# wkgcass/vproxy

Measured on AMD Instinct MI355X. Metric: device-resident GB/s, batched IPv4+TCP checksum, 1500B pkts, 1/2/4/8 GPU, higher is better.
Workload: dtype u8

## Files before the change

vproxy_amd/csrc/tcp_build.hip:

```cpp
#include <hip/hip_runtime.h>
#include <stdint.h>

#include "device_common.h"
#include "internal.h"
#include "tcp_build.h"
#include "team_move.h"

namespace vpcsum {

__global__ __launch_bounds__(256) void k_tcp_build(uint8_t* __restrict__ dst, uint64_t dst_len,
                                                  const uint8_t* __restrict__ src, uint64_t src_len,
                                                  const vpcsum_tcphdr_t* __restrict__ hdrs, uint32_t n_hdr,
                                                  const vpcsum_tcpseg_t* __restrict__ segs, uint32_t n,
                                                  uint32_t* __restrict__ frame_len_out, uint32_t* __restrict__ out,
                                                  uint8_t* __restrict__ status) {
    const uint32_t tid = blockIdx.x * 256u + threadIdx.x;
    const uint32_t i = tid >> 3;
    const uint32_t tl = threadIdx.x & 7u;
    if (i >= n) return;

    const u32x4a4_t ra = *(gu32x4a4_t*)(segs + i);
    const u32x4a4_t rb = *(gu32x4a4_t*)((const uint8_t*)(segs + i) + 16);
    const uint64_t frame_off = ((uint64_t)ra.y << 32) | ra.x, data_off = ((uint64_t)ra.w << 32) | ra.z;
    const uint32_t seq = rb.x, hdr = rb.y, frame_cap = rb.z;
    const uint32_t data_len = rb.w & 0xffffu, flags = (rb.w >> 16) & 0xffu, rsv = rb.w >> 24;

    bool ok = tcp_build_seg_ok(hdr, n_hdr, flags, rsv);
    uint32_t t[16] = {0, 0, 0, 0, 0, 0, 0, 0, 0, 0, 0, 0, 0, 0, 0, 0};
    if (ok) {
        const uint8_t* hp = (const uint8_t*)(hdrs + hdr);
        const u32x4a4_t h0 = *(gu32x4a4_t*)hp, h1 = *(gu32x4a4_t*)(hp + 16), h2 = *(gu32x4a4_t*)(hp + 32),
                        h3 = *(gu32x4a4_t*)(hp + 48);
        t[0] = h0.x; t[1] = h0.y; t[2] = h0.z; t[3] = h0.w;
        t[4] = h1.x; t[5] = h1.y; t[6] = h1.z; t[7] = h1.w;
        t[8] = h2.x; t[9] = h2.y; t[10] = h2.z; t[11] = h2.w;
        t[12] = h3.x; t[13] = h3.y; t[14] = h3.z; t[15] = h3.w;
        ok = tcp_build_hdr_ok(t) && tcp_build_fits(t, frame_off, data_off, frame_cap, data_len, dst_len, src_len);
    }
    if (!ok) {
        if (tl == 0) {
            frame_len_out[i] = 0u;
            if (out) out[i] = 0u;
            if (status) status[i] = (uint8_t)VPCSUM_S_BAD_DESC;
        }
        return;
    }

    const bool v4 = tb_l3_ver(t) == 4;
    const uint32_t l2 = tb_l2_len(t), H = tcp_build_header_len(t);
    uint8_t* const frame = dst + frame_off;
    uint8_t* const pay = frame + H;

    const Span sp = make_span((uintptr_t)pay, (uintptr_t)(src + data_off), data_len, 0u);
    const uint32_t ng = data_len ? (sp.hi + 15u) >> 4 : 0u;
    const uint64_t acc = move_groups<false>(sp, tl, ng);
    uint32_t ps = fold32(team_sum<8>(fold64(acc)));
    if ((uintptr_t)pay & 1u) ps = bswap16(ps);

    TcpBuildWords w;
    tcp_build_words(t, seq, data_len, flags, w);
    const uint32_t ip_field = v4 ? 0xffffu - fold64(tcp_build_ip_header_sum(w)) : 0u;
    const uint32_t l4_field = 0xffffu - fold64(tcp_build_l4_header_sum(t, w, data_len) + ps);
    tcp_build_set_sums(w, v4, ip_field, l4_field);

    if (tl == 0) {
        if (l2) {
            store_piece_any<14>(frame, Piece{w.eth[0], w.eth[1], w.eth[2], w.eth[3], 0u});
        }
        frame_len_out[i] = H + data_len;
        if (out) out[i] = bswap16(ip_field) | (bswap16(l4_field) << 16);
        if (status) status[i] = (uint8_t)VPCSUM_S_DONE;
    } else if (tl == 1) {
        store_piece_any<20>(frame + l2, Piece{w.ip[0], w.ip[1], w.ip[2], w.ip[3], w.ip[4]});
    } else if (tl == 2 && !v4) {
        store_piece_any<20>(frame + l2 + 20u, Piece{w.ip[5], w.ip[6], w.ip[7], w.ip[8], w.ip[9]});
    } else if (tl == (v4 ? 2u : 3u)) {
        store_piece_any<20>(frame + l2 + (v4 ? 20u : 40u), Piece{w.tcp[0], w.tcp[1], w.tcp[2], w.tcp[3], w.tcp[4]});
    }
}

hipError_t launch_tcp_build(uint8_t* dst, uint64_t dst_len, const uint8_t* src, uint64_t src_len,
                            const vpcsum_tcphdr_t* hdrs, uint32_t n_hdr, const vpcsum_tcpseg_t* segs, uint32_t n,
                            uint32_t* frame_len_out, uint32_t* out, uint8_t* status, hipStream_t stream) {
    if (n == 0) return hipSuccess;
    const uint32_t g = (n + 31u) / 32u;
    hipLaunchKernelGGL(k_tcp_build, dim3(g), dim3(256), 0, stream, dst, dst_len, src, src_len, hdrs, n_hdr, segs, n,
                       frame_len_out, out, status);
    return hipGetLastError();
}

}
```

vproxy_amd/csrc/tcp_recv.hip:

```cpp
#include <hip/hip_runtime.h>
#include <stdint.h>

#include "device_common.h"
#include "internal.h"
#include "tcp_recv.h"
#include "team_move.h"

namespace vpcsum {

namespace {

__device__ __forceinline__ uint32_t load_shifted(uintptr_t p) {
    const uint32_t sh = (uint32_t)p & 3u;
    const uintptr_t a = p - sh;
    const uint32_t lo = *(gu32_t*)a;
    const uint32_t hi = sh ? *(gu32_t*)(a + 4) : 0u;
    return alignbyte(hi, lo, sh);
}

struct Desc {
    uint64_t l3_off;
    uint32_t l3_len, l4_off, l3_ver, l4_proto, flags;
};
__device__ __forceinline__ Desc load_desc(const vpcsum_desc_t* d) {
    const u32x4a4_t v = *(gu32x4a4_t*)d;
    Desc r;
    r.l3_off = ((uint64_t)v.y << 32) | v.x;
    r.l3_len = v.z & 0xffffu;
    r.l4_off = v.z >> 16;
    r.l3_ver = v.w & 0xffu;
    r.l4_proto = (v.w >> 8) & 0xffu;
    r.flags = (v.w >> 16) & 0xffu;
    return r;
}

}

__global__ __launch_bounds__(256) void k_tcp_recv(const uint8_t* __restrict__ arena, uint64_t arena_len,
                                                 const vpcsum_desc_t* __restrict__ desc,
                                                 const vpcsum_tcprx_t* __restrict__ rx, uint32_t n,
                                                 uint8_t* __restrict__ dst, uint64_t dst_len,
                                                 uint32_t* __restrict__ stored_out, uint32_t* __restrict__ out,
                                                 uint8_t* __restrict__ status) {
    const uint32_t tid = blockIdx.x * 256u + threadIdx.x;
    const uint32_t i = tid >> 3;
    const uint32_t tl = threadIdx.x & 7u;
    if (i >= n) return;

    const Desc d = load_desc(desc + i);
    const u32x4a4_t ra = *(gu32x4a4_t*)(rx + i);
    const uint64_t dst_off = ((uint64_t)ra.y << 32) | ra.x;
    const uint32_t dst_cap = ra.z, skip = ra.w & 0xffffu, ops = (ra.w >> 16) & 0xffu, rsv = ra.w >> 24;

    bool ok = tcp_recv_desc_ok(d.l3_off, d.l3_len, d.l4_off, d.l3_ver, d.l4_proto, d.flags, arena_len) &&
              tcp_recv_ops_ok(ops, rsv);
    const uint32_t seg_len = d.l3_len - d.l4_off;
    const uintptr_t l3 = (uintptr_t)arena + d.l3_off, seg = l3 + d.l4_off;
    uint32_t hlen = 0, data_len = 0, stored = 0;
    if (ok) {
        const uint32_t b12 = *(gu8_t*)(seg + 12);
        ok = tcp_recv_hdr_ok(seg_len, b12, &hlen, &data_len) &&
             tcp_recv_store_ok(data_len, skip, ops, dst_off, dst_cap, dst_len, &stored);
    }
    if (!ok) {
        if (tl == 0) {
            stored_out[i] = 0u;
            if (out) out[i] = 0u;
            if (status) status[i] = (uint8_t)VPCSUM_S_BAD_DESC;
        }
        return;
    }
    const uint32_t field = (uint32_t) * (gu8_t*)(seg + 16) | ((uint32_t) * (gu8_t*)(seg + 17) << 8);

    const uintptr_t v0 = stored ? (uintptr_t)dst + dst_off - (hlen + skip) : seg;
    const Span sp = make_span(v0, seg, seg_len, stored ? hlen + skip : seg_len);
    const uint32_t ng = (sp.hi + 15u) >> 4;
    const uint64_t acc = move_groups<true>(sp, tl, ng);

    const bool v4 = d.l3_ver == 4u;
    uint32_t ph = 0;
    if (tl < (v4 ? 2u : 8u)) {
        const uint32_t w = load_shifted(l3 + (v4 ? 12u : 8u) + 4u * tl);
        ph = (w & 0xffffu) + (w >> 16);
    }
    uint32_t ipw = 0;
    if (tl == 7u && (d.flags & VPCSUM_F_IP)) {
        const uint32_t sh = (uint32_t)l3 & 3u, nw = d.l4_off >> 2;
        const uintptr_t a = l3 - sh;
        uint64_t ipacc = 0;
        uint32_t cur = *(gu32_t*)a, ip_field = 0;
        for (uint32_t j = 0; j < nw; ++j) {
            const uint32_t nxt = (sh || j + 1u < nw) ? *(gu32_t*)(a + 4u * j + 4u) : 0u;
            uint32_t w = alignbyte(nxt, cur, sh);
            cur = nxt;
            if (j == 2u) {
                ip_field = w >> 16;
                w &= 0xffffu;
            }
            ipacc += w;
        }
        const uint32_t ipc = 0xffffu - bswap16(fold64(ipacc));
        ipw = ipc | (bswap16(ip_field) == ipc ? 0x10000u : 0u);
    }

    uint32_t ps = fold32(team_sum<8>(fold64(acc)));
    if (v0 & 1u) ps = bswap16(ps);
    ph = team_sum<8>(ph);
    ipw = team_sum<8>(ipw);
    if (tl == 0) {
        const uint64_t total = (uint64_t)ps + ph + (6u << 8) + bswap16(seg_len) + (0xffffu - field);
        const uint32_t l4c = 0xffffu - bswap16(fold64(total));
        uint32_t st = VPCSUM_S_DONE;
        if (bswap16(field) == l4c) st |= VPCSUM_S_L4_OK;
        if (ipw & 0x10000u) st |= VPCSUM_S_IP_OK;
        stored_out[i] = stored;
        if (out) out[i] = (ipw & 0xffffu) | (l4c << 16);
        if (status) status[i] = (uint8_t)st;
    }
}

__global__ __launch_bounds__(256) void k_tcp_digest(const uint8_t* __restrict__ arena, uint64_t arena_len,
                                                   const vpcsum_desc_t* __restrict__ desc, uint32_t n,
                                                   vpcsum_tcpinfo_t* __restrict__ info) {
    const uint32_t i = blockIdx.x * 256u + threadIdx.x;
    if (i >= n) return;
    const Desc d = load_desc(desc + i);
    u32x4_t o;
    o.x = o.y = o.z = o.w = 0u;
    if (tcp_recv_desc_ok(d.l3_off, d.l3_len, d.l4_off, d.l3_ver, d.l4_proto, d.flags, arena_len)) {
        const uintptr_t seg = (uintptr_t)arena + d.l3_off + d.l4_off;
        const uint32_t sh = (uint32_t)seg & 3u;
        const uintptr_t a = seg - sh;
        const u32x4a4_t v = *(gu32x4a4_t*)a;
        const uint32_t w4 = sh ? *(gu32_t*)(a + 16) : 0u;
        const uint32_t d1 = alignbyte(v.z, v.y, sh), d2 = alignbyte(v.w, v.z, sh),
                       d3 = alignbyte(w4, v.w, sh);
        uint32_t hlen = 0, data_len = 0;
        if (tcp_recv_hdr_ok(d.l3_len - d.l4_off, d3 & 0xffu, &hlen, &data_len)) {
            o.x = __builtin_bswap32(d1);
            o.y = __builtin_bswap32(d2);
            o.z = bswap16(d3 >> 16) | (data_len << 16);
            o.w = hlen | (((d3 >> 8) & 0x3fu) << 8);
        }
    }
    *(gwu32x4_t*)(info + i) = o;
}

hipError_t launch_tcp_recv(const uint8_t* arena, uint64_t arena_len, const vpcsum_desc_t* desc, const vpcsum_tcprx_t* rx,
                           uint32_t n, uint8_t* dst, uint64_t dst_len, uint32_t* stored, uint32_t* out, uint8_t* status,
                           hipStream_t stream) {
    if (n == 0) return hipSuccess;
    const uint32_t g = (n + 31u) / 32u;
    hipLaunchKernelGGL(k_tcp_recv, dim3(g), dim3(256), 0, stream, arena, arena_len, desc, rx, n, dst, dst_len, stored, out,
                       status);
    return hipGetLastError();
}

hipError_t launch_tcp_digest(const uint8_t* arena, uint64_t arena_len, const vpcsum_desc_t* desc, uint32_t n,
                             vpcsum_tcpinfo_t* info, hipStream_t stream) {
    if (n == 0) return hipSuccess;
    hipLaunchKernelGGL(k_tcp_digest, dim3((n + 255u) / 256u), dim3(256), 0, stream, arena, arena_len, desc, n, info);
    return hipGetLastError();
}

}
```

vproxy_amd/csrc/team_move.h:

```cpp
#pragma once
#include <stdint.h>

#include "device_common.h"

#define VPC_TM_FN __host__ __device__ __forceinline__

namespace vpcsum {

#ifdef __HIP_DEVICE_COMPILE__
#define VPC_TM_LOAD(T, a) __builtin_nontemporal_load((T*)(a))
VPC_TM_FN uint32_t alignbyte(uint32_t hi, uint32_t lo, uint32_t sh) { return __builtin_amdgcn_alignbyte(hi, lo, sh); }
#else
#define VPC_TM_LOAD(T, a) (*(T*)(a))
VPC_TM_FN uint32_t alignbyte(uint32_t hi, uint32_t lo, uint32_t sh) {
    return (uint32_t)((((uint64_t)hi << 32) | lo) >> ((sh & 3u) * 8u));
}
#endif

struct Span {
    uintptr_t sa;
    uintptr_t pd;
    uint32_t sh;
    uint32_t lo, hi;
    uint32_t s_lo, s_hi;
    uint32_t k_lo, k_hi;
};

VPC_TM_FN Span make_span(uintptr_t v0, uintptr_t seg, uint32_t seg_len, uint32_t store_from) {
    Span sp;
    sp.lo = (uint32_t)v0 & 15u;
    sp.hi = sp.lo + seg_len;
    sp.pd = v0 - sp.lo;
    sp.s_lo = sp.lo + store_from;
    sp.s_hi = sp.hi;
    const uintptr_t s0 = seg - sp.lo;
    sp.sh = (uint32_t)s0 & 3u;
    sp.sa = s0 - sp.sh;
    sp.k_lo = (sp.lo + sp.sh) >> 2;
    sp.k_hi = (sp.lo + sp.sh + seg_len - 1u) >> 2;
    return sp;
}

struct Group {
    uint32_t w0, w1, w2, w3, w4;
};

VPC_TM_FN bool group_inner(const Span& sp, uint32_t g) { return g * 16u >= sp.lo && g * 16u + 16u <= sp.hi; }

VPC_TM_FN Group load_group(const Span& sp, uint32_t g) {
    Group r;
    const uintptr_t q = sp.sa + (size_t)g * 16u;
    if (group_inner(sp, g)) {
        const u32x4a4_t v = VPC_TM_LOAD(gu32x4a4_t, q);
        r.w0 = v.x; r.w1 = v.y; r.w2 = v.z; r.w3 = v.w;
        r.w4 = sp.sh ? VPC_TM_LOAD(gu32_t, q + 16) : 0u;
    } else {
        const uint32_t k = g * 4u;
        r.w0 = (k >= sp.k_lo && k <= sp.k_hi) ? VPC_TM_LOAD(gu32_t, q) : 0u;
        r.w1 = (k + 1 >= sp.k_lo && k + 1 <= sp.k_hi) ? VPC_TM_LOAD(gu32_t, q + 4) : 0u;
        r.w2 = (k + 2 >= sp.k_lo && k + 2 <= sp.k_hi) ? VPC_TM_LOAD(gu32_t, q + 8) : 0u;
        r.w3 = (k + 3 >= sp.k_lo && k + 3 <= sp.k_hi) ? VPC_TM_LOAD(gu32_t, q + 12) : 0u;
        r.w4 = (k + 4 >= sp.k_lo && k + 4 <= sp.k_hi) ? VPC_TM_LOAD(gu32_t, q + 16) : 0u;
    }
    return r;
}

VPC_TM_FN void store_partial(uintptr_t a, uint32_t v, uint32_t m) {
    if ((m & 0xffffu) == 0xffffu) {
        *(gwu16_t*)a = (uint16_t)v;
    } else {
        if (m & 0xffu) *(gwu8_t*)a = (uint8_t)v;
        if (m & 0xff00u) *(gwu8_t*)(a + 1) = (uint8_t)(v >> 8);
    }
    if ((m >> 16) == 0xffffu) {
        *(gwu16_t*)(a + 2) = (uint16_t)(v >> 16);
    } else {
        if (m & 0xff0000u) *(gwu8_t*)(a + 2) = (uint8_t)(v >> 16);
        if (m & 0xff000000u) *(gwu8_t*)(a + 3) = (uint8_t)(v >> 24);
    }
}

template <bool SUB>
VPC_TM_FN void emit_group(const Span& sp, uint32_t g, const Group& r, uint64_t& acc) {
    uint32_t d0 = alignbyte(r.w1, r.w0, sp.sh);
    uint32_t d1 = alignbyte(r.w2, r.w1, sp.sh);
    uint32_t d2 = alignbyte(r.w3, r.w2, sp.sh);
    uint32_t d3 = alignbyte(r.w4, r.w3, sp.sh);
    const uint32_t rel = g * 16u;
    const uintptr_t p = sp.pd + (size_t)rel;
    const uint32_t s_lo = SUB ? sp.s_lo : sp.lo, s_hi = SUB ? sp.s_hi : sp.hi;
    if (rel >= s_lo && rel + 16u <= s_hi) {
        acc += (uint64_t)d0 + d1 + d2 + d3;
        u32x4_t o;
        o.x = d0; o.y = d1; o.z = d2; o.w = d3;
        *(gwu32x4_t*)p = o;
        return;
    }
    if (!SUB || !group_inner(sp, g)) {
        const int lo = (int)sp.lo, hi = (int)sp.hi;
        d0 &= bmask((int)rel, lo, hi);
        d1 &= bmask((int)rel + 4, lo, hi);
        d2 &= bmask((int)rel + 8, lo, hi);
        d3 &= bmask((int)rel + 12, lo, hi);
    }
    acc += (uint64_t)d0 + d1 + d2 + d3;
    if (!SUB || (rel + 16u > s_lo && rel < s_hi)) {
        const int lo = (int)s_lo, hi = (int)s_hi;
        const uint32_t m0 = bmask((int)rel, lo, hi), m1 = bmask((int)rel + 4, lo, hi), m2 = bmask((int)rel + 8, lo, hi),
                       m3 = bmask((int)rel + 12, lo, hi);
        if (m0 == 0xffffffffu) *(gwu32_t*)p = d0; else if (m0) store_partial(p, d0, m0);
        if (m1 == 0xffffffffu) *(gwu32_t*)(p + 4) = d1; else if (m1) store_partial(p + 4, d1, m1);
        if (m2 == 0xffffffffu) *(gwu32_t*)(p + 8) = d2; else if (m2) store_partial(p + 8, d2, m2);
        if (m3 == 0xffffffffu) *(gwu32_t*)(p + 12) = d3; else if (m3) store_partial(p + 12, d3, m3);
    }
}

template <bool SUB>
VPC_TM_FN uint64_t move_groups(const Span& sp, uint32_t tl, uint32_t ng) {
    uint64_t acc = 0;
    for (uint32_t g = tl; g < ng; g += 16u) {
        const bool two = g + 8u < ng;
        const Group a = load_group(sp, g);
        Group b = {0u, 0u, 0u, 0u, 0u};
        if (two) b = load_group(sp, g + 8u);
        emit_group<SUB>(sp, g, a, acc);
        if (two) emit_group<SUB>(sp, g + 8u, b, acc);
    }
    return acc;
}


struct Piece {
    uint32_t w0, w1, w2, w3, w4;
};

template <int K>
__device__ __forceinline__ uint32_t piece_word(const Piece w) {
    return K == 0 ? w.w0 : K == 1 ? w.w1 : K == 2 ? w.w2 : K == 3 ? w.w3 : K == 4 ? w.w4 : 0u;
}

template <int POS>
__device__ __forceinline__ uint32_t piece_bytes(const Piece w) {
    constexpr int k = POS >> 2, sh = (POS & 3) * 8;
    const uint32_t lo = piece_word<k>(w);
    if constexpr (sh == 0) return lo;
    else return (lo >> sh) | (piece_word<k + 1>(w) << (32 - sh));
}

template <int R, int NB, int POS = 0>
__device__ __forceinline__ void store_piece(uint8_t* p, const Piece w) {
    if constexpr (POS < NB) {
        constexpr int a = (R + POS) & 3;
        if constexpr (a == 0 && NB - POS >= 4) {
            *(gwu32_t*)(p + POS) = piece_bytes<POS>(w);
            store_piece<R, NB, POS + 4>(p, w);
        } else if constexpr ((a & 1) == 0 && NB - POS >= 2) {
            *(gwu16_t*)(p + POS) = (uint16_t)piece_bytes<POS>(w);
            store_piece<R, NB, POS + 2>(p, w);
        } else {
            *(gwu8_t*)(p + POS) = (uint8_t)piece_bytes<POS>(w);
            store_piece<R, NB, POS + 1>(p, w);
        }
    }
}

template <int NB>
__device__ __forceinline__ void store_piece_any(uint8_t* p, const Piece w) {
    switch ((uint32_t)(uintptr_t)p & 3u) {
    case 0: store_piece<0, NB>(p, w); break;
    case 1: store_piece<1, NB>(p, w); break;
    case 2: store_piece<2, NB>(p, w); break;
    default: store_piece<3, NB>(p, w); break;
    }
}

}
```

Before: 6814.

## Deepen team move loop and share neighbor words via DPP instead of reloads

The team copy/checksum loop now loads four 16-byte groups per lane per iteration instead of two, so more loads are in flight. For misaligned spans, the extra trailing word each lane used to load is taken from the neighbouring lane's first word with DPP lane shifts. The span base is aligned to 64 bytes instead of 16. In tcp_build, the header stores are issued before the payload move, and the TCP checksum is OR'd into the final TCP header word. This adds register pressure and relies on the DPP row-shift semantics matching the 8-lane team layout, which is a correctness risk.

```diff
diff --git a/vproxy_amd/csrc/tcp_build.hip b/vproxy_amd/csrc/tcp_build.hip
--- a/vproxy_amd/csrc/tcp_build.hip
+++ b/vproxy_amd/csrc/tcp_build.hip
@@ -51,31 +51,32 @@
     uint8_t* const frame = dst + frame_off;
     uint8_t* const pay = frame + H;
 
-    const Span sp = make_span((uintptr_t)pay, (uintptr_t)(src + data_off), data_len, 0u);
-    const uint32_t ng = data_len ? (sp.hi + 15u) >> 4 : 0u;
-    const uint64_t acc = move_groups<false>(sp, tl, ng);
-    uint32_t ps = fold32(team_sum<8>(fold64(acc)));
-    if ((uintptr_t)pay & 1u) ps = bswap16(ps);
-
     TcpBuildWords w;
     tcp_build_words(t, seq, data_len, flags, w);
     const uint32_t ip_field = v4 ? 0xffffu - fold64(tcp_build_ip_header_sum(w)) : 0u;
-    const uint32_t l4_field = 0xffffu - fold64(tcp_build_l4_header_sum(t, w, data_len) + ps);
-    tcp_build_set_sums(w, v4, ip_field, l4_field);
-
+    const uint32_t l4_head = fold64(tcp_build_l4_header_sum(t, w, data_len));
+    tcp_build_set_sums(w, v4, ip_field, 0u);
     if (tl == 0) {
-        if (l2) {
-            store_piece_any<14>(frame, Piece{w.eth[0], w.eth[1], w.eth[2], w.eth[3], 0u});
-        }
-        frame_len_out[i] = H + data_len;
-        if (out) out[i] = bswap16(ip_field) | (bswap16(l4_field) << 16);
-        if (status) status[i] = (uint8_t)VPCSUM_S_DONE;
+        if (l2) store_piece_any<14>(frame, Piece{w.eth[0], w.eth[1], w.eth[2], w.eth[3], 0u});
     } else if (tl == 1) {
         store_piece_any<20>(frame + l2, Piece{w.ip[0], w.ip[1], w.ip[2], w.ip[3], w.ip[4]});
     } else if (tl == 2 && !v4) {
         store_piece_any<20>(frame + l2 + 20u, Piece{w.ip[5], w.ip[6], w.ip[7], w.ip[8], w.ip[9]});
+    }
+
+    const Span sp = make_span((uintptr_t)pay, (uintptr_t)(src + data_off), data_len, 0u);
+    const uint32_t ng = data_len ? (sp.hi + 15u) >> 4 : 0u;
+    const uint64_t acc = move_groups<false, kMoveDepth>(sp, tl, ng);
+    uint32_t ps = fold32(team_sum<8>(fold64(acc)));
+    if ((uintptr_t)pay & 1u) ps = bswap16(ps);
+    const uint32_t l4_field = 0xffffu - fold64((uint64_t)l4_head + ps);
+
+    if (tl == 0) {
+        frame_len_out[i] = H + data_len;
+        if (out) out[i] = bswap16(ip_field) | (bswap16(l4_field) << 16);
+        if (status) status[i] = (uint8_t)VPCSUM_S_DONE;
     } else if (tl == (v4 ? 2u : 3u)) {
-        store_piece_any<20>(frame + l2 + (v4 ? 20u : 40u), Piece{w.tcp[0], w.tcp[1], w.tcp[2], w.tcp[3], w.tcp[4]});
+        store_piece_any<20>(pay - 20, Piece{w.tcp[0], w.tcp[1], w.tcp[2], w.tcp[3], w.tcp[4] | l4_field});
     }
 }
 
diff --git a/vproxy_amd/csrc/tcp_recv.hip b/vproxy_amd/csrc/tcp_recv.hip
--- a/vproxy_amd/csrc/tcp_recv.hip
+++ b/vproxy_amd/csrc/tcp_recv.hip
@@ -75,7 +75,7 @@
     const uintptr_t v0 = stored ? (uintptr_t)dst + dst_off - (hlen + skip) : seg;
     const Span sp = make_span(v0, seg, seg_len, stored ? hlen + skip : seg_len);
     const uint32_t ng = (sp.hi + 15u) >> 4;
-    const uint64_t acc = move_groups<true>(sp, tl, ng);
+    const uint64_t acc = move_groups<true, kMoveDepth>(sp, tl, ng);
 
     const bool v4 = d.l3_ver == 4u;
     uint32_t ph = 0;
diff --git a/vproxy_amd/csrc/team_move.h b/vproxy_amd/csrc/team_move.h
--- a/vproxy_amd/csrc/team_move.h
+++ b/vproxy_amd/csrc/team_move.h
@@ -17,6 +17,8 @@
 }
 #endif
 
+constexpr int kMoveDepth = 4;
+
 struct Span {
     uintptr_t sa;
     uintptr_t pd;
@@ -28,7 +30,7 @@
 
 VPC_TM_FN Span make_span(uintptr_t v0, uintptr_t seg, uint32_t seg_len, uint32_t store_from) {
     Span sp;
-    sp.lo = (uint32_t)v0 & 15u;
+    sp.lo = (uint32_t)v0 & 63u;
     sp.hi = sp.lo + seg_len;
     sp.pd = v0 - sp.lo;
     sp.s_lo = sp.lo + store_from;
@@ -47,13 +49,13 @@
 
 VPC_TM_FN bool group_inner(const Span& sp, uint32_t g) { return g * 16u >= sp.lo && g * 16u + 16u <= sp.hi; }
 
-VPC_TM_FN Group load_group(const Span& sp, uint32_t g) {
+VPC_TM_FN Group load_group(const Span& sp, uint32_t g, bool own_w4) {
     Group r;
     const uintptr_t q = sp.sa + (size_t)g * 16u;
     if (group_inner(sp, g)) {
         const u32x4a4_t v = VPC_TM_LOAD(gu32x4a4_t, q);
         r.w0 = v.x; r.w1 = v.y; r.w2 = v.z; r.w3 = v.w;
-        r.w4 = sp.sh ? VPC_TM_LOAD(gu32_t, q + 16) : 0u;
+        r.w4 = (sp.sh && own_w4) ? VPC_TM_LOAD(gu32_t, q + 16) : 0u;
     } else {
         const uint32_t k = g * 4u;
         r.w0 = (k >= sp.k_lo && k <= sp.k_hi) ? VPC_TM_LOAD(gu32_t, q) : 0u;
@@ -63,6 +65,16 @@
         r.w4 = (k + 4 >= sp.k_lo && k + 4 <= sp.k_hi) ? VPC_TM_LOAD(gu32_t, q + 16) : 0u;
     }
     return r;
+}
+
+VPC_TM_FN uint32_t next_group_w0(const Span& sp, uint32_t g, uint32_t tl, uint32_t same, uint32_t next, bool take) {
+#ifdef __HIP_DEVICE_COMPILE__
+    const uint32_t a = (uint32_t)__builtin_amdgcn_update_dpp(0, (int)same, 0x101, 0xF, 0xF, false);
+    const uint32_t b = (uint32_t)__builtin_amdgcn_update_dpp(0, (int)next, 0x117, 0xF, 0xF, false);
+    return tl < 7u ? a : b;
+#else
+    return take ? VPC_TM_LOAD(gu32_t, sp.sa + (size_t)g * 16u + 16u) : 0u;
+#endif
 }
 
 VPC_TM_FN void store_partial(uintptr_t a, uint32_t v, uint32_t m) {
@@ -115,16 +127,26 @@
     }
 }
 
-template <bool SUB>
+template <bool SUB, int D = kMoveDepth>
 VPC_TM_FN uint64_t move_groups(const Span& sp, uint32_t tl, uint32_t ng) {
     uint64_t acc = 0;
-    for (uint32_t g = tl; g < ng; g += 16u) {
-        const bool two = g + 8u < ng;
-        const Group a = load_group(sp, g);
-        Group b = {0u, 0u, 0u, 0u, 0u};
-        if (two) b = load_group(sp, g + 8u);
-        emit_group<SUB>(sp, g, a, acc);
-        if (two) emit_group<SUB>(sp, g + 8u, b, acc);
+    for (uint32_t g = tl; g < ng; g += 8u * D) {
+        Group r[D];
+        bool nb[D];
+#pragma unroll
+        for (int j = 0; j < D; ++j) {
+            const uint32_t gj = g + 8u * j;
+            nb[j] = sp.sh && (tl < 7u || j + 1 < D) && group_inner(sp, gj) && group_inner(sp, gj + 1u);
+            r[j] = Group{0u, 0u, 0u, 0u, 0u};
+            if (gj < ng) r[j] = load_group(sp, gj, !nb[j]);
+        }
+#pragma unroll
+        for (int j = 0; j < D; ++j) {
+            const uint32_t gj = g + 8u * j;
+            const uint32_t w = next_group_w0(sp, gj, tl, r[j].w0, j + 1 < D ? r[j + 1].w0 : 0u, nb[j]);
+            if (nb[j]) r[j].w4 = w;
+            if (gj < ng) emit_group<SUB>(sp, gj, r[j], acc);
+        }
     }
     return acc;
 }
```

Result: no change. 6813 (-0.0%).
